# leaner-forever/SEGS-SLAM

Measured on AMD Instinct MI355X. Metric: mapper train-iters/sec (fwd+bwd raster), higher is better.
Workload: dtype f32; 1 GPU; 1080p_3m: 3000000 Gaussians, 1920x1080, 1 keyframe per GPU, fwd+bwd raster; P=3000000, P_visible=2096178, num_rendered=10472370, instances_binned=7913347, instances_live=6766534, width=1920, height=1080, parallelism=keyframe-dp1, forward=resident (no host sync), hipgraph=off

## Files before the change

### segs-slam_amd/csrc/binning.hip

```cpp
#include <hip/hip_runtime.h>
#include <cstdint>
#include "gs_layout.h"
#include "kernels.h"

namespace segs {

constexpr int PREFIX_ROWS = PREFIX_ROWS_PER_WG;

__global__ void __launch_bounds__(1024) scan_block_sums_kernel(uint32_t* __restrict__ block_sums, int nblocks,
                                                               const uint32_t* __restrict__ depth_range,
                                                               uint32_t* __restrict__ total) {
  __shared__ uint32_t w_sum[16], w_dmax[16], w_dnmin[16];
  const int tid = threadIdx.x, lane = tid & 63, wv = tid >> 6;
  uint32_t sum = 0, dmax = 0, dnmin = 0;
  for (int i = tid; i < nblocks; i += 1024) {
    sum += block_sums[i];
    dmax = max(dmax, depth_range[i]);
    dnmin = max(dnmin, depth_range[nblocks + i]);
  }
#pragma unroll
  for (int off = 32; off > 0; off >>= 1) {
    sum += __shfl_down(sum, off, 64);
    dmax = max(dmax, (uint32_t)__shfl_down((int)dmax, off, 64));
    dnmin = max(dnmin, (uint32_t)__shfl_down((int)dnmin, off, 64));
// ... 49 lines not shown
  __syncthreads();
  uint32_t carry = red[0] + red[1] + red[2] + red[3];
  uint32_t vals[PREFIX_ROWS];
#pragma unroll
  for (int r = 0; r < PREFIX_ROWS; r++) {
    const uint32_t slot = slot0 + (uint32_t)r * 256u + tid;
    vals[r] = slot < (uint32_t)P ? incl[slot] : 0u;
  }
#pragma unroll
  for (int r = 0; r < PREFIX_ROWS; r++) {
    const uint32_t slot = slot0 + (uint32_t)r * 256u + tid;
    uint32_t x = vals[r];
    const uint32_t t0 = x;
#pragma unroll
    for (int off = 1; off < 64; off <<= 1) {
      uint32_t y = __shfl_up(x, off, 64);
      if (lane >= off) x += y;
    }
    __syncthreads();
    if (lane == 63) wave_tot[wv] = x;
    __syncthreads();
    uint32_t base = carry;
    for (int w = 0; w < wv; w++) base += wave_tot[w];
    const uint32_t v = base + x;
    if (slot < (uint32_t)P) incl[slot] = v;
    if (slot < (uint32_t)P && first_owner && t0 != 0u) {
      const uint32_t excl = v - t0;
      for (uint32_t k = (excl + EMIT_SLOTS_PER_WG - 1) / EMIT_SLOTS_PER_WG; k * EMIT_SLOTS_PER_WG < v && k < owner_entries; k++)
        first_owner[k] = slot;
    }
    carry += wave_tot[0] + wave_tot[1] + wave_tot[2] + wave_tot[3];
  }
  if (total_out && blockIdx.x == gridDim.x - 1 && tid == 0) total_out[0] = carry;
}

constexpr int EMIT_SLOTS = EMIT_SLOTS_PER_WG;
static_assert(EMIT_SLOTS == 2 * 256, "two consecutive slots per thread");
struct EmitLds {
  uint32_t excl[EMIT_SLOTS + 2];
  uint32_t idx[EMIT_SLOTS + 1];
  uint2 bin[EMIT_SLOTS + 1];
  float4 geo0[EMIT_SLOTS + 1];
  float2 geo1[EMIT_SLOTS + 1];
  uint32_t mark[EMIT_SLOTS];
  uint32_t wave_max[4];
};
constexpr uint32_t EMIT_OWNER_MASK = 1023u;

__device__ __forceinline__ void emit_stage_owner(EmitLds& L, int k, uint32_t idx, const float4& e0, const float4& e1) {
  const uint32_t rmin = __float_as_uint(e1.z), rmax = __float_as_uint(e1.w);
  L.idx[k] = idx;
  L.bin[k] = make_uint2(rmin, (rmax & 0xFFFFu) - (rmin & 0xFFFFu));
  const float op = e1.y;
  L.geo0[k] = make_float4(e0.x, e0.y, -e0.z, -0.5f * e0.w);
  L.geo1[k] = make_float2(-e1.x, (op * 255.0f > 1.0f) ? __builtin_amdgcn_logf(255.0f * op) * 1.0001f + 1e-3f : -1.0f);
}
__device__ __forceinline__ void emit_mark_owner(uint32_t* mark, int k, uint32_t start, uint32_t s0, uint32_t tag) {
  const uint32_t pos = start > s0 ? start - s0 : 0u;
  if (pos < (uint32_t)EMIT_SLOTS) mark[pos] = (tag << 10) | (uint32_t)k;
}
__device__ __forceinline__ void emit_scan_begin(EmitLds& L, const uint32_t* mark, int tid, uint32_t& m0, uint32_t& incl) {
  const uint2 m = *reinterpret_cast<const uint2*>(mark + 2 * tid);
  m0 = m.x;
  uint32_t x = max(m.x, m.y);
#pragma unroll
  for (int off = 1; off < 64; off <<= 1) {
// ... 359 lines not shown
      if (AUX) aux_out[gp] = s_aux[lp];
      if constexpr (sizeof(K) == 4) {
        if (ranges_out != nullptr) {
          const K prev = lp > 0 ? s_keys[lp - 1] : ~k, next = lp + 1 < nout ? s_keys[lp + 1] : ~k;
          if (k != prev) atomicMin(&ranges_out[k].x, (uint32_t)gp);
          if (k != next) atomicMax(&ranges_out[k].y, (uint32_t)gp + 1u);
        }
      }
    }
  }
}

#define SEGS_INSTANTIATE_RADIX(K, BITS)                                                                                          \
  template __global__ void radix_count_kernel<K, BITS>(const K*, int, int, uint32_t, int, uint32_t*, uint32_t*, int, int,       \
                                                       const uint32_t*, int, int, int);                                                  \
  template __global__ void radix_scatter_kernel<K, BITS, false>(const K*, const uint32_t*, K*, uint32_t*, int, int, uint32_t, int, \
                                                                const uint32_t*, const uint32_t*, const uint32_t*, int, int,        \
                                                                const uint32_t*, int, uint32_t*, const uint32_t*, uint32_t*, int, int, int, \
                                                                uint2*, uint32_t*, uint32_t*, int);
SEGS_INSTANTIATE_RADIX(uint64_t, 8)
SEGS_INSTANTIATE_RADIX(uint32_t, 8)
SEGS_INSTANTIATE_RADIX(uint32_t, 9)
SEGS_INSTANTIATE_RADIX(uint32_t, 11)
#undef SEGS_INSTANTIATE_RADIX
#define SEGS_INSTANTIATE_AUX(BITS)                                                                                                     \
  template __global__ void radix_scatter_kernel<uint32_t, BITS, true>(const uint32_t*, const uint32_t*, uint32_t*, uint32_t*, int, int, \
                                                                      uint32_t, int, const uint32_t*, const uint32_t*, const uint32_t*, \
                                                                      int, int, const uint32_t*, int, uint32_t*, const uint32_t*, uint32_t*, int, int, int, \
                                                                      uint2*, uint32_t*, uint32_t*, int);
SEGS_INSTANTIATE_AUX(8)
SEGS_INSTANTIATE_AUX(9)
#undef SEGS_INSTANTIATE_AUX

__global__ void __launch_bounds__(256) identify_tile_ranges_kernel(int L, const uint32_t* __restrict__ keys,
                                                                   uint2* __restrict__ ranges, const uint32_t* __restrict__ n_dev,
                                                                   uint32_t* __restrict__ status, uint32_t* __restrict__ status_mirror,
                                                                   const uint32_t* __restrict__ n_live ) {
  static_assert(RANGE_KEYS_PER_THREAD == 4, "one uint4 per thread");
  const int idx = blockIdx.x * 256 + threadIdx.x;
  if (n_dev) {
    const uint32_t n = *n_dev;
    if (idx == 0 && status) {
      const uint32_t over = (n > (uint32_t)L || status[2] != 0u) ? 1u : 0u;
      status[2] = 0u;
      status[3] = over;
      const uint32_t live = n_live ? min(*n_live, min(n, (uint32_t)L)) : min(n, (uint32_t)L);
      status[1] = live;
      if (status_mirror) { status_mirror[0] = n; status_mirror[1] = live; status_mirror[3] = over; }
    }
    L = (int)min(n, (uint32_t)L);
  }
  if (n_live) L = (int)min(*n_live, (uint32_t)L);
  const int i0 = idx * RANGE_KEYS_PER_THREAD;
  if (i0 >= L) return;
  uint32_t k[RANGE_KEYS_PER_THREAD];
  if (i0 + RANGE_KEYS_PER_THREAD <= L) {
    const uint4 v = *reinterpret_cast<const uint4*>(keys + i0);
    k[0] = v.x; k[1] = v.y; k[2] = v.z; k[3] = v.w;
  } else {
#pragma unroll
    for (int q = 0; q < RANGE_KEYS_PER_THREAD; q++) k[q] = i0 + q < L ? keys[i0 + q] : 0u;
  }
  uint32_t prev = i0 > 0 ? keys[i0 - 1] : 0u;
#pragma unroll
  for (int q = 0; q < RANGE_KEYS_PER_THREAD; q++) {
    const int i = i0 + q;
// ... 120 lines not shown
```

### segs-slam_amd/csrc/capi.hip

```cpp
#include <hip/hip_runtime.h>
#include <cstdio>
#include <cstdlib>
#include <algorithm>
#include <cstring>
#include <string>
#include <vector>
#include "../../include/segs_raster.h"
#include "gs_layout.h"
#include "kernels.h"

using namespace segs;

namespace {
thread_local std::string g_err;
}
int segs::set_error(int code, const char* what) {
  g_err = what;
  return code;
}
int segs::set_hip_error(hipError_t e, const char* where) {
  g_err = std::string(where) + ": " + hipGetErrorString(e);
  return (int)e > 0 ? (int)e : 1;
}

namespace {

thread_local uint32_t g_flags = 0u;
thread_local uint32_t* g_status_mirror = nullptr;

int fail(int code, const char* what) { return segs::set_error(code, what); }
int hip_fail(hipError_t e, const char* where) { return segs::set_hip_error(e, where); }
#define HIP_TRY(expr)                                   \
  do {                                                  \
    hipError_t _e = (expr);                             \
    if (_e != hipSuccess) return hip_fail(_e, #expr);   \
  } while (0)
#define LAUNCH_TRY(name)                                \
  do {                                                  \
    hipError_t _e = hipGetLastError();                  \
    if (_e != hipSuccess) return hip_fail(_e, name);    \
  } while (0)

enum KernelId { K_PREPROCESS_FWD = 0, K_SCAN, K_DUPLICATE, K_RADIX_COUNT, K_RADIX_SCAN, K_RADIX_SCATTER, K_RANGES,
                K_RENDER_FWD, K_RENDER_BWD, K_PREPROCESS_BWD, K_MEMSET, K_COUNT };
const char* const kKernelNames[K_COUNT] = {"preprocess_fwd_kernel", "scan_block_sums_kernel", "duplicate_with_keys_kernel",
                                           "radix_count_kernel", "radix_scan_kernel", "radix_scatter_kernel",
                                           "identify_tile_ranges_kernel", "render_fwd_kernel", "render_bwd_kernel",
                                           "preprocess_bwd_kernel", "memset"};
struct Profiler {
  unsigned mask = 0;
  std::vector<hipEvent_t> pool;
  size_t used = 0;
  struct Span { int id; size_t e0, e1; };
  std::vector<Span> spans;
  double total_ms[K_COUNT] = {0};
  long count[K_COUNT] = {0};
  hipEvent_t get() {
    if (used == pool.size()) { hipEvent_t e; if (hipEventCreate(&e) != hipSuccess) return nullptr; pool.push_back(e); }
    return pool[used++];
  }
} g_prof;
struct ProfScope {
  int id; hipStream_t st; size_t e0 = 0; bool on;
  ProfScope(int id_, hipStream_t st_) : id(id_), st(st_), on((g_prof.mask >> id_) & 1u) {
    if (on) { e0 = g_prof.used; hipEvent_t e = g_prof.get(); if (e) (void)hipEventRecord(e, st); else on = false; }
  }
  ~ProfScope() {
    if (on) { size_t e1 = g_prof.used; hipEvent_t e = g_prof.get(); if (e) { (void)hipEventRecord(e, st); g_prof.spans.push_back({id, e0, e1}); } }
  }
};
#define PROF(id) ProfScope _prof_scope_##id(id, st)

uint32_t getHigherMsb(uint32_t n) {
  uint32_t msb = sizeof(n) * 4, step = msb;
  while (step > 1) {
    step /= 2;
    if (n >> msb) msb += step; else msb -= step;
  }
  if (n >> msb) msb++;
  return msb;
}
// ... 86 lines not shown
  float* gacc() const { return (float*)(base + L.gacc); }
  uint32_t* touched() const { return (uint32_t*)(base + L.touched); }
};
Geom geom_at(char* p, int P) { return Geom{geom_layout(P), align_ptr(p)}; }
Geom geom_at(char* p, int P, int rows) {
  Geom g{geom_layout(rows), align_ptr(p)};
  g.L.P = P;
  g.L.nblocks = (P + 255) / 256;
  return g;
}

int run_preprocess(const Geom& G, int P, int W, int H, const float* means3D, const float* colors, const float* opac,
                   const float* scales, float mod, const float* rots, const float* cov3D_precomp, const float* view,
                   const float* proj, float tan_fovx, float tan_fovy, int* radii, const float* shs, int D, int M,
                   const float* cam_pos, hipStream_t st, uint32_t* depth_keys = nullptr, uint32_t* depth_vals = nullptr,
                   uint2* ranges = nullptr, uint32_t extra_flags = 0u, uint32_t* depth_overflow = nullptr) {
  const float focal_y = H / (2.0f * tan_fovy);
  const float focal_x = W / (2.0f * tan_fovx);
  const uint32_t gx = (W + TILE_X - 1) / TILE_X, gy = (H + TILE_Y - 1) / TILE_Y;
  { PROF(K_PREPROCESS_FWD);
  preprocess_fwd_kernel<<<G.L.nblocks, 256, 0, st>>>(P, means3D, scales, mod, rots, opac, colors, cov3D_precomp, view,
                                                     proj, W, H, tan_fovx, tan_fovy, focal_x, focal_y, gx, gy, radii,
                                                     G.rec(), G.bin(), G.block_sums(), G.block_sums() + (G.L.nblocks + 1), shs, D, M, cam_pos,
                                                     G.clamped(), g_flags | extra_flags, depth_keys, depth_vals, ranges, (int)(gx * gy),
                                                     depth_overflow, G.touched());
  }
  LAUNCH_TRY("preprocess_fwd_kernel");
  return SEGS_OK;
}

int run_binning(const Geom& G, char* bin, const BinningLayout& BL, const GaussSortLayout& GS, uint2* ranges, int P, int n_cap,
                const uint32_t* n_dev, uint32_t dmin, int dbits, uint32_t dcull, uint32_t gx, uint32_t gy, uint32_t* total_out,
                hipStream_t st, bool depth_keys_ready = false, bool drop_dead = false, bool nine_bit_depth = false,
                const uint32_t* depth_keys_src = nullptr ) {
  const int bit = (int)getHigherMsb(gx * gy);
  char* gbin = bin + GS.base;
  const BinningLayout& GL = GS.inner;
  const int gside = (nine_bit_depth ? (dbits + 8) / 9 : (dbits + 7) / 8) & 1;
  if (!depth_keys_ready) { PROF(K_DUPLICATE);
  make_depth_keys_kernel<<<G.L.nblocks, 256, 0, st>>>(P, G.bin(), dcull, (uint32_t*)(gbin + GL.keys[gside]), (uint32_t*)(gbin + GL.vals[gside]),
                                                      ranges, (int)(gx * gy));
  }
  LAUNCH_TRY("make_depth_keys_kernel");
  const bool drop_culled = depth_keys_ready;
  int idx_bits = 1;
  while (idx_bits < 32 && ((uint64_t)1 << idx_bits) < (uint64_t)P) idx_bits++;
  int pack_shift = (32 - idx_bits >= 6 && !(g_flags & SEGS_RASTER_GATHER_TILES_TOUCHED)) ? idx_bits : 0;
  if (pack_shift && (g_flags & SEGS_RASTER_TEST_NARROW_PACK)) pack_shift = 30;
  uint32_t* aux_final = pack_shift ? nullptr : G.offsets();
  int rc = nine_bit_depth ? sort_pairs<uint32_t, 9>(gbin, GL, P, dbits, dmin, dbits, st, nullptr, drop_culled, true, G.touched(), aux_final, pack_shift, SortFusion(), depth_keys_src)
                          : sort_pairs<uint32_t>(gbin, GL, P, dbits, dmin, dbits, st, nullptr, drop_culled, true, G.touched(), aux_final, pack_shift, SortFusion(), depth_keys_src);
  if (rc) return rc;
  uint32_t* order = (uint32_t*)(gbin + GL.vals[0]);
  const uint32_t* ng_dev = drop_culled ? (const uint32_t*)(gbin + GL.n_live) : nullptr;
  uint32_t* sums2 = (uint32_t*)(bin + GS.block_sums);
  uint32_t* first_owner = (uint32_t*)(bin + GS.first_owner);
  const int prefix_wgs = (P + 256 * PREFIX_ROWS_PER_WG - 1) / (256 * PREFIX_ROWS_PER_WG);
  { PROF(K_SCAN);
  ordered_block_sums_kernel<<<prefix_wgs, 256, 0, st>>>(P, pack_shift ? G.touched() : G.offsets(), nullptr, sums2, G.offsets(), ng_dev, order, pack_shift);
  }
  LAUNCH_TRY("ordered_block_sums_kernel");
#ifdef SEGS_MEASURE
  static const bool no_wide = getenv("SEGS_NO_WIDE_DIGIT") != nullptr;
#else
  constexpr bool no_wide = false;
#endif
  const bool wide_digit = !no_wide && bit <= 11 && BL.nblocks <= SORT_WIDE_MAX_TILES;
  const int tpasses = wide_digit ? 1 : (bit + 7) / 8;
  const int side = tpasses & 1;
  { PROF(K_SCAN);
  ordered_offsets_kernel<<<prefix_wgs, 256, 0, st>>>(P, sums2, G.offsets(), total_out, ng_dev, first_owner,
                                                      (uint32_t)(n_cap / EMIT_SLOTS_PER_WG + 2));
  }
  LAUNCH_TRY("ordered_offsets_kernel");
  const bool unfused = (g_flags & SEGS_RASTER_UNFUSED_BINNING) != 0u;
  { PROF(K_DUPLICATE);
  duplicate_with_keys_kernel<<<(n_cap + EMIT_SLOTS_PER_WG - 1) / EMIT_SLOTS_PER_WG, 256, 0, st>>>(P, n_cap, G.rec(), order, G.offsets(),
                                                                    (uint32_t*)(bin + BL.keys[side]), (uint32_t*)(bin + BL.vals[side]), gx, n_dev,
                                                                    drop_dead ? 1 : 0, ng_dev, first_owner);
  }
  LAUNCH_TRY("duplicate_with_keys_kernel");
  SortFusion fuse;
  const bool fused_ranges = !unfused && tpasses >= 2;
  if (fused_ranges) {
    fuse.ranges = ranges;
    fuse.status = n_dev ? total_out : nullptr;
    fuse.status_mirror = n_dev ? g_status_mirror : nullptr;
    fuse.keep_sorted_keys = n_dev == nullptr;
  }
  rc = wide_digit ? sort_pairs<uint32_t, 11>(bin, BL, n_cap, bit, 0u, 0, st, n_dev, drop_dead, false, nullptr, nullptr, 0, fuse)
                  : sort_pairs<uint32_t>(bin, BL, n_cap, bit, 0u, 0, st, n_dev, drop_dead, false, nullptr, nullptr, 0, fuse);
  if (rc) return rc;
  if (!fused_ranges) { PROF(K_RANGES);
  identify_tile_ranges_kernel<<<(n_cap + 256 * RANGE_KEYS_PER_THREAD - 1) / (256 * RANGE_KEYS_PER_THREAD), 256, 0, st>>>(n_cap, (const uint32_t*)(bin + BL.keys[0]), ranges, n_dev,
                                                                   n_dev ? total_out : nullptr, n_dev ? g_status_mirror : nullptr,
                                                                   drop_dead ? (const uint32_t*)(bin + BL.n_live) : nullptr);
  }
  LAUNCH_TRY("identify_tile_ranges_kernel");
  return SEGS_OK;
}

int launch_render_fwd(uint32_t tiles, const uint2* ranges, const uint32_t* point_list, int width, int height, const float* rec,
                      const float* background, float* final_T, uint32_t* n_contrib, float* out_color, const segs_depth_outputs* dout,
                      hipStream_t st) {
  PROF(K_RENDER_FWD);
  if (dout && (dout->depth || dout->alpha))
    render_fwd_depth_kernel<<<tiles, 256, 0, st>>>(ranges, point_list, width, height, rec, background, final_T, n_contrib, out_color,
                                                   dout->depth, dout->alpha);
  else
    render_fwd_kernel<<<tiles, 256, 0, st>>>(ranges, point_list, width, height, rec, background, final_T, n_contrib, out_color);
  LAUNCH_TRY("render_fwd_kernel");
  return SEGS_OK;
}

}

extern "C" {

const char* segs_last_error(void) { return g_err.c_str(); }

uint32_t* segs_raster_set_status_mirror(uint32_t* host_mapped_status) {
  uint32_t* old = g_status_mirror;
  g_status_mirror = host_mapped_status;
  return old;
}

uint32_t segs_raster_set_flags(uint32_t flags) {
  const uint32_t old = g_flags;
  g_flags = flags;
  return old;
}
// ... 395 lines not shown
                                    const float* background, int width, int height, const float* means3D, const float* shs,
                                    const float* colors_precomp, const float* opacities, const float* scales, float scale_modifier,
                                    const float* rotations, const float* cov3D_precomp, const float* viewmatrix,
                                    const float* projmatrix, const float* cam_pos, float tan_fovx, float tan_fovy, float* out_color,
                                    int* radii, uint32_t* status, const segs_depth_outputs* dout, void* stream) {
  hipStream_t st = (hipStream_t)stream;
  if (P <= 0 || capacity <= 0 || width <= 0 || height <= 0) return fail(SEGS_ERR_INVALID_ARGUMENT, "bad sizes");
  if (geom_rows < P) return fail(SEGS_ERR_INVALID_ARGUMENT, "geom_rows (rows the geometry buffer was sized for) must be >= P");
  if (geom_rows > MAX_GAUSSIANS) return fail(SEGS_ERR_INVALID_ARGUMENT, "P exceeds 2^28 Gaussians");
  if (!geom_buffer || !binning_buffer || !image_buffer || !status || !background || !out_color || !viewmatrix || !projmatrix ||
      !means3D || !opacities)
    return fail(SEGS_ERR_INVALID_ARGUMENT, "null required pointer");
  if (!colors_precomp && (!shs || !cam_pos || M <= 0 || D < 0 || (D + 1) * (D + 1) > M || D > 3))
    return fail(SEGS_ERR_INVALID_ARGUMENT, "need colors_precomp, or shs + cam_pos with (D+1)^2 <= M, D <= 3");
  if (!cov3D_precomp && (!scales || !rotations)) return fail(SEGS_ERR_INVALID_ARGUMENT, "need scales+rotations or cov3D_precomp");
  const uint32_t gx = (width + TILE_X - 1) / TILE_X, gy = (height + TILE_Y - 1) / TILE_Y;
  if (gx > 0xFFFFu || gy > 0xFFFFu) return fail(SEGS_ERR_INVALID_ARGUMENT, "image too large for 16-bit tile coordinates");
  Geom G = geom_at(geom_buffer, P, geom_rows);
  char* img = align_ptr(image_buffer);
  char* bin = align_ptr(binning_buffer);
  const ImageLayout IL = image_layout(width, height);
  const BinningLayout BL = binning_layout(capacity);
  const GaussSortLayout GS = gauss_sort_layout(capacity, P);
  if (!radii) radii = G.radii_internal();
  uint2* ranges = (uint2*)(img + IL.ranges);
  char* gbin = bin + GS.base;
  const int gside = (3 & 1);
  int rc = run_preprocess(G, P, width, height, means3D, colors_precomp, opacities, cov3D_precomp ? nullptr : scales, scale_modifier,
                          rotations, cov3D_precomp, viewmatrix, projmatrix, tan_fovx, tan_fovy, radii, shs, D, M, cam_pos, st,
                          (uint32_t*)(gbin + GS.inner.keys[gside]), (uint32_t*)(gbin + GS.inner.vals[gside]), ranges,
                          (g_flags & SEGS_RASTER_KEEP_DEAD_INSTANCES) ? 0u : PREPROCESS_TIGHT_RECT, status + 2);
  if (rc) return rc;
  rc = run_binning(G, bin, BL, GS, ranges, P, capacity, status, DEPTH_KEY_MIN, DEPTH_KEY_BITS, 0xFFFFFFFFu, gx, gy, status, st, true,
                   (g_flags & SEGS_RASTER_KEEP_DEAD_INSTANCES) == 0u, true);
  if (rc) return rc;
  return launch_render_fwd(gx * gy, ranges, (const uint32_t*)(bin + BL.vals[0]), width, height, G.rec(), background,
                           (float*)(img + IL.final_T), (uint32_t*)(img + IL.n_contrib), out_color, dout, st);
}

int segs_rasterize_forward_resident(char* geom_buffer, char* binning_buffer, char* image_buffer, int capacity, int geom_rows, int P, int D, int M,
                                    const float* background, int width, int height, const float* means3D, const float* shs,
                                    const float* colors_precomp, const float* opacities, const float* scales, float scale_modifier,
                                    const float* rotations, const float* cov3D_precomp, const float* viewmatrix,
                                    const float* projmatrix, const float* cam_pos, float tan_fovx, float tan_fovy, float* out_color,
                                    int* radii, uint32_t* status, void* stream) {
  return rasterize_forward_resident_impl(geom_buffer, binning_buffer, image_buffer, capacity, geom_rows, P, D, M, background, width, height,
                                         means3D, shs, colors_precomp, opacities, scales, scale_modifier, rotations, cov3D_precomp,
                                         viewmatrix, projmatrix, cam_pos, tan_fovx, tan_fovy, out_color, radii, status, nullptr, stream);
}

int segs_rasterize_forward_resident_depth(char* geom_buffer, char* binning_buffer, char* image_buffer, int capacity, int geom_rows, int P,
                                          int D, int M, const float* background, int width, int height, const float* means3D,
                                          const float* shs, const float* colors_precomp, const float* opacities, const float* scales,
                                          float scale_modifier, const float* rotations, const float* cov3D_precomp,
                                          const float* viewmatrix, const float* projmatrix, const float* cam_pos, float tan_fovx,
                                          float tan_fovy, float* out_color, int* radii, uint32_t* status,
                                          const segs_depth_outputs* depth_out, void* stream) {
  return rasterize_forward_resident_impl(geom_buffer, binning_buffer, image_buffer, capacity, geom_rows, P, D, M, background, width, height,
                                         means3D, shs, colors_precomp, opacities, scales, scale_modifier, rotations, cov3D_precomp,
                                         viewmatrix, projmatrix, cam_pos, tan_fovx, tan_fovy, out_color, radii, status, depth_out, stream);
}

int segs_resident_projection_targets(char* geom_buffer, char* binning_buffer, char* image_buffer, int capacity, int geom_rows, int P,
                                     int width, int height, int* radii, uint32_t* status, segs_projection_targets* out) {
  if (P <= 0 || capacity <= 0 || width <= 0 || height <= 0 || !out) return fail(SEGS_ERR_INVALID_ARGUMENT, "bad sizes");
  if (geom_rows < P) return fail(SEGS_ERR_INVALID_ARGUMENT, "geom_rows (rows the geometry buffer was sized for) must be >= P");
  if (geom_rows > MAX_GAUSSIANS) return fail(SEGS_ERR_INVALID_ARGUMENT, "P exceeds 2^28 Gaussians");
// ... 4 lines not shown
  const ImageLayout IL = image_layout(width, height);
  const GaussSortLayout GS = gauss_sort_layout(capacity, P);
  const int gside = (3 & 1);
  out->records = G.rec();
  out->radii = radii ? radii : G.radii_internal();
  out->tiles_touched = G.touched();
  out->depth_keys = (uint32_t*)(align_ptr(binning_buffer) + GS.base + GS.inner.keys[gside]);
  out->tile_ranges = (uint32_t*)(align_ptr(image_buffer) + IL.ranges);
  out->depth_overflow = status + 2;
  out->num_tiles = (int)(gx * gy);
  out->flags = (g_flags & SEGS_RASTER_KEEP_DEAD_INSTANCES) ? 0u : PREPROCESS_TIGHT_RECT;
  return SEGS_OK;
}

static int rasterize_forward_resident_projected_impl(char* geom_buffer, char* binning_buffer, char* image_buffer, int capacity,
                                                    int geom_rows, int P, const float* background, int width, int height, float* out_color,
                                                    uint32_t* status, const segs_depth_outputs* dout, void* stream) {
  hipStream_t st = (hipStream_t)stream;
  if (P <= 0 || capacity <= 0 || width <= 0 || height <= 0) return fail(SEGS_ERR_INVALID_ARGUMENT, "bad sizes");
  if (geom_rows < P) return fail(SEGS_ERR_INVALID_ARGUMENT, "geom_rows (rows the geometry buffer was sized for) must be >= P");
  if (geom_rows > MAX_GAUSSIANS) return fail(SEGS_ERR_INVALID_ARGUMENT, "P exceeds 2^28 Gaussians");
  if (!geom_buffer || !binning_buffer || !image_buffer || !status || !background || !out_color)
    return fail(SEGS_ERR_INVALID_ARGUMENT, "null required pointer");
  const uint32_t gx = (width + TILE_X - 1) / TILE_X, gy = (height + TILE_Y - 1) / TILE_Y;
  if (gx > 0xFFFFu || gy > 0xFFFFu) return fail(SEGS_ERR_INVALID_ARGUMENT, "image too large for 16-bit tile coordinates");
  Geom G = geom_at(geom_buffer, P, geom_rows);
  char* img = align_ptr(image_buffer);
  char* bin = align_ptr(binning_buffer);
  const ImageLayout IL = image_layout(width, height);
  const BinningLayout BL = binning_layout(capacity);
  const GaussSortLayout GS = gauss_sort_layout(capacity, P);
  uint2* ranges = (uint2*)(img + IL.ranges);
  int rc = run_binning(G, bin, BL, GS, ranges, P, capacity, status, DEPTH_KEY_MIN, DEPTH_KEY_BITS, 0xFFFFFFFFu, gx, gy, status, st, true,
                       (g_flags & SEGS_RASTER_KEEP_DEAD_INSTANCES) == 0u, true);
  if (rc) return rc;
  return launch_render_fwd(gx * gy, ranges, (const uint32_t*)(bin + BL.vals[0]), width, height, G.rec(), background,
                           (float*)(img + IL.final_T), (uint32_t*)(img + IL.n_contrib), out_color, dout, st);
}

int segs_rasterize_forward_resident_projected(char* geom_buffer, char* binning_buffer, char* image_buffer, int capacity, int geom_rows, int P,
                                              const float* background, int width, int height, float* out_color, uint32_t* status,
                                              void* stream) {
  return rasterize_forward_resident_projected_impl(geom_buffer, binning_buffer, image_buffer, capacity, geom_rows, P, background, width,
                                                   height, out_color, status, nullptr, stream);
}

int segs_rasterize_forward_resident_projected_depth(char* geom_buffer, char* binning_buffer, char* image_buffer, int capacity,
                                                    int geom_rows, int P, const float* background, int width, int height,
                                                    float* out_color, uint32_t* status, const segs_depth_outputs* depth_out,
                                                    void* stream) {
  return rasterize_forward_resident_projected_impl(geom_buffer, binning_buffer, image_buffer, capacity, geom_rows, P, background, width,
                                                   height, out_color, status, depth_out, stream);
}

int segs_rasterize_backward_resident(char* geom_buffer, char* binning_buffer, char* image_buffer, int capacity, int geom_rows, int P, int D, int M,
                                     const float* background, int width, int height, const float* means3D, const float* shs,
                                     const float* scales, float scale_modifier, const float* rotations, const float* cov3D_precomp,
                                     const float* viewmatrix, const float* projmatrix, const float* campos, float tan_fovx,
                                     float tan_fovy, const int* radii, const float* dL_dpix, float* dL_dmean2D, float* dL_dconic,
                                     float* dL_dopacity, float* dL_dcolor, float* dL_dmean3D, float* dL_dcov3D, float* dL_dsh,
                                     float* dL_dscale, float* dL_drot, void* stream) {
  return rasterize_backward_impl(P, D, M, capacity, background, width, height, means3D, shs, scales, scale_modifier, rotations,
                                 cov3D_precomp, viewmatrix, projmatrix, campos, tan_fovx, tan_fovy, radii, geom_buffer, binning_buffer,
                                 image_buffer, dL_dpix, dL_dmean2D, dL_dconic, dL_dopacity, dL_dcolor, dL_dmean3D, dL_dcov3D, dL_dsh,
                                 dL_dscale, dL_drot, stream, true, geom_rows, nullptr);
}

// ... 40 lines not shown
```

### segs-slam_amd/csrc/kernels.h

```cpp
#pragma once
#include <hip/hip_runtime.h>
#include <cstdint>
#include "gs_layout.h"

namespace segs {

int set_error(int code, const char* what);
int set_hip_error(hipError_t e, const char* where);


__global__ void preprocess_fwd_kernel(
    int P, const float* __restrict__ means3D, const float* __restrict__ scales, float mod,
    const float* __restrict__ rotations, const float* __restrict__ opacities, const float* __restrict__ colors,
    const float* __restrict__ cov3D_precomp, const float* __restrict__ viewmatrix, const float* __restrict__ projmatrix,
    int W, int H, float tan_fovx, float tan_fovy, float focal_x, float focal_y, uint32_t gx, uint32_t gy,
    int* __restrict__ radii, float* __restrict__ rec, BinInfo* __restrict__ bin, uint32_t* __restrict__ block_sums,
    uint32_t* __restrict__ depth_range, const float* __restrict__ shs, int D, int M, const float* __restrict__ cam_pos,
    uint32_t* __restrict__ clamped, uint32_t flags, uint32_t* __restrict__ depth_keys, uint32_t* __restrict__ depth_vals,
    uint2* __restrict__ ranges, int num_tiles, uint32_t* __restrict__ depth_overflow, uint32_t* __restrict__ touched_dense);
constexpr uint32_t DEPTH_KEY_MIN = 0x3E4CCCCDu;
constexpr int DEPTH_KEY_BITS = 27;

__global__ void visible_filter_kernel(
    int P, const float* __restrict__ means3D, const float* __restrict__ scales, float mod,
    const float* __restrict__ rotations, const float* __restrict__ cov3D_precomp,
    const float* __restrict__ viewmatrix, const float* __restrict__ projmatrix, int W, int H,
    float tan_fovx, float tan_fovy, float focal_x, float focal_y, uint32_t gx, uint32_t gy, int* __restrict__ radii,
    int log_scale_stride);

__global__ void mark_visible_kernel(int P, const float* __restrict__ means3D, const float* __restrict__ viewmatrix,
                                    uint8_t* __restrict__ present);

template <bool DEPTH>
__global__ void preprocess_bwd_kernel(
    int P, const float* __restrict__ means3D, const int* __restrict__ radii, const float* __restrict__ scales,
    const float* __restrict__ rotations, float mod, const float* __restrict__ cov3D_precomp,
    const float* __restrict__ view, const float* __restrict__ proj, float h_x, float h_y, float tan_fovx, float tan_fovy,
    float* __restrict__ gacc, float img_w, float img_h,
    float* __restrict__ dL_dmean2D, float* __restrict__ dL_dconic,
    float* __restrict__ dL_dopacity, float* __restrict__ dL_dcolor, float* __restrict__ dL_dmean3D,
    float* __restrict__ dL_dcov3D, float* __restrict__ dL_dscale, float* __restrict__ dL_drot, int clean_gacc);
__global__ void sh_backward_kernel(int P, const float* __restrict__ means3D, const int* __restrict__ radii,
                                   const float* __restrict__ shs, int D, int M, const float* __restrict__ cam_pos,
                                   const uint32_t* __restrict__ clamped, const float* __restrict__ dL_dcolor,
                                   float* __restrict__ dL_dmean3D, float* __restrict__ dL_dsh);

__global__ void scan_block_sums_kernel(uint32_t* __restrict__ block_sums, int nblocks, const uint32_t* __restrict__ depth_range,
                                       uint32_t* __restrict__ total);
__global__ void ordered_offsets_kernel(int P, const uint32_t* __restrict__ block_sums, uint32_t* __restrict__ incl,
                                       uint32_t* __restrict__ total_out, const uint32_t* __restrict__ ng_dev,
                                       uint32_t* __restrict__ first_owner, uint32_t owner_entries);
__global__ void duplicate_with_keys_kernel(int P, int R, const float* __restrict__ rec,
                                           const uint32_t* __restrict__ order, const uint32_t* __restrict__ incl,
                                           uint32_t* __restrict__ keys, uint32_t* __restrict__ vals, uint32_t gx,
                                           const uint32_t* __restrict__ n_dev, int mark_dead, const uint32_t* __restrict__ ng_dev,
                                           const uint32_t* __restrict__ first_owner);
constexpr uint32_t RANGE_EMPTY_START = 0xFFFFFFFFu;
__global__ void normalize_ranges_kernel(int num_tiles, uint2* __restrict__ ranges);
constexpr uint32_t PREPROCESS_TIGHT_RECT = 0x80000000u;
constexpr uint32_t DEAD_KEY = 0xFFFFFFFFu;
template <typename K, int BITS>
__global__ void radix_count_kernel(const K* __restrict__ keys, int n, int shift, uint32_t dmin, int dbits,
                                   uint32_t* __restrict__ tile_prefix, uint32_t* __restrict__ chunk_hist, int nblocks, int nchunks,
                                   const uint32_t* __restrict__ n_dev, int drop_dead, int chunk_tiles, int nbits);
__global__ void radix_scan_kernel(uint32_t* __restrict__ block_hist, int nblocks, uint32_t* __restrict__ digit_totals);
template <typename K, int BITS, bool AUX>
__global__ void radix_scatter_kernel(const K* __restrict__ keys_in, const uint32_t* __restrict__ vals_in,
                                     K* __restrict__ keys_out, uint32_t* __restrict__ vals_out, int n, int shift,
                                     uint32_t dmin, int dbits, const uint32_t* __restrict__ tile_prefix, const uint32_t* __restrict__ chunk_prefix,
                                     const uint32_t* __restrict__ digit_totals, int nblocks, int nchunks,
                                     const uint32_t* __restrict__ n_dev, int drop_dead, uint32_t* __restrict__ n_live_out,
                                     const uint32_t* __restrict__ aux_in, uint32_t* __restrict__ aux_out, int nbits, int chunk_tiles, int pack_shift,
                                     uint2* __restrict__ ranges_out, uint32_t* __restrict__ status, uint32_t* __restrict__ status_mirror,
                                     int write_keys);
__global__ void identify_tile_ranges_kernel(int L, const uint32_t* __restrict__ keys, uint2* __restrict__ ranges,
                                            const uint32_t* __restrict__ n_dev, uint32_t* __restrict__ status,
                                            uint32_t* __restrict__ status_mirror, const uint32_t* __restrict__ n_live);

__global__ void render_fwd_kernel(const uint2* __restrict__ ranges, const uint32_t* __restrict__ point_list, int W, int H,
                                  const float* __restrict__ rec, const float* __restrict__ bg,
                                  float* __restrict__ final_T, uint32_t* __restrict__ n_contrib, float* __restrict__ out_color);
__global__ void render_bwd_kernel(const uint2* __restrict__ ranges, const uint32_t* __restrict__ point_list, int W, int H,
                                  const float* __restrict__ rec, const float* __restrict__ bg,
                                  const float* __restrict__ final_T, const uint32_t* __restrict__ n_contrib,
// ... 32 lines not shown
```

Measured before the change: 1002 iters/s.

## Replace global depth sort with index-order binning plus per-tile depth sort

Instead of radix-sorting all visible Gaussians by depth before duplication, Gaussians are compacted in index order with a fused count/offset scan. After tile binning, a new kernel sorts each tile's instance list by depth in LDS, using a chunked merge-rank path for large tiles. This removes the global depth sort passes in exchange for per-tile sorting work and extra key gathers, which may be imbalanced on heavy tiles.

New measurement: 1016 iters/s, median of 6. +1.3%, better.

```diff
diff --git a/segs-slam_amd/csrc/binning.hip b/segs-slam_amd/csrc/binning.hip
--- a/segs-slam_amd/csrc/binning.hip
+++ b/segs-slam_amd/csrc/binning.hip
@@ -105,6 +105,75 @@
     carry += wave_tot[0] + wave_tot[1] + wave_tot[2] + wave_tot[3];
   }
   if (total_out && blockIdx.x == gridDim.x - 1 && tid == 0) total_out[0] = carry;
+}
+
+__global__ void __launch_bounds__(256) index_block_sums_kernel(int P, const uint32_t* __restrict__ touched,
+                                                               uint32_t* __restrict__ block_sums, uint32_t* __restrict__ block_owners) {
+  __shared__ uint32_t wave_sums[4], wave_owners[4];
+  uint32_t s = 0, c = 0;
+#pragma unroll
+  for (int r = 0; r < PREFIX_ROWS; r++) {
+    const int g = (blockIdx.x * PREFIX_ROWS + r) * 256 + threadIdx.x;
+    const uint32_t v = g < P ? touched[g] : 0u;
+    s += v;
+    c += v != 0u ? 1u : 0u;
+  }
+#pragma unroll
+  for (int off = 32; off > 0; off >>= 1) { s += __shfl_down(s, off, 64); c += __shfl_down(c, off, 64); }
+  if ((threadIdx.x & 63) == 0) { wave_sums[threadIdx.x >> 6] = s; wave_owners[threadIdx.x >> 6] = c; }
+  __syncthreads();
+  if (threadIdx.x == 0) {
+    block_sums[blockIdx.x] = wave_sums[0] + wave_sums[1] + wave_sums[2] + wave_sums[3];
+    block_owners[blockIdx.x] = wave_owners[0] + wave_owners[1] + wave_owners[2] + wave_owners[3];
+  }
+}
+__global__ void __launch_bounds__(256) index_offsets_kernel(int P, const uint32_t* __restrict__ touched, const uint32_t* __restrict__ block_sums,
+                                                            const uint32_t* __restrict__ block_owners, uint32_t* __restrict__ order,
+                                                            uint32_t* __restrict__ incl, uint32_t* __restrict__ total_out, uint32_t* __restrict__ ng_out,
+                                                            uint32_t* __restrict__ first_owner, uint32_t owner_entries) {
+  __shared__ uint32_t wave_tot[4], wave_cnt[4], red[4], red_c[4];
+  const int tid = threadIdx.x, lane = tid & 63, wv = tid >> 6;
+  uint32_t before = 0, before_c = 0;
+  for (int b = tid; b < (int)blockIdx.x; b += 256) { before += block_sums[b]; before_c += block_owners[b]; }
+#pragma unroll
+  for (int off = 32; off > 0; off >>= 1) { before += __shfl_down(before, off, 64); before_c += __shfl_down(before_c, off, 64); }
+  if (lane == 0) { red[wv] = before; red_c[wv] = before_c; }
+  __syncthreads();
+  uint32_t carry = red[0] + red[1] + red[2] + red[3], carry_c = red_c[0] + red_c[1] + red_c[2] + red_c[3];
+  const int g0 = blockIdx.x * 256 * PREFIX_ROWS;
+  uint32_t vals[PREFIX_ROWS];
+#pragma unroll
+  for (int r = 0; r < PREFIX_ROWS; r++) {
+    const int g = g0 + r * 256 + tid;
+    vals[r] = g < P ? touched[g] : 0u;
+  }
+#pragma unroll
+  for (int r = 0; r < PREFIX_ROWS; r++) {
+    const int g = g0 + r * 256 + tid;
+    const uint32_t t0 = vals[r];
+    uint32_t x = t0, c = t0 != 0u ? 1u : 0u;
+#pragma unroll
+    for (int off = 1; off < 64; off <<= 1) {
+      const uint32_t y = __shfl_up(x, off, 64), yc = __shfl_up(c, off, 64);
+      if (lane >= off) { x += y; c += yc; }
+    }
+    __syncthreads();
+    if (lane == 63) { wave_tot[wv] = x; wave_cnt[wv] = c; }
+    __syncthreads();
+    uint32_t base = carry, base_c = carry_c;
+    for (int w = 0; w < wv; w++) { base += wave_tot[w]; base_c += wave_cnt[w]; }
+    if (t0 != 0u) {
+      const uint32_t v = base + x, slot = base_c + c - 1u;
+      order[slot] = (uint32_t)g;
+      incl[slot] = v;
+      const uint32_t excl = v - t0;
+      for (uint32_t k = (excl + EMIT_SLOTS_PER_WG - 1) / EMIT_SLOTS_PER_WG; k * EMIT_SLOTS_PER_WG < v && k < owner_entries; k++)
+        first_owner[k] = slot;
+    }
+    carry += wave_tot[0] + wave_tot[1] + wave_tot[2] + wave_tot[3];
+    carry_c += wave_cnt[0] + wave_cnt[1] + wave_cnt[2] + wave_cnt[3];
+  }
+  if (blockIdx.x == gridDim.x - 1 && tid == 0) { total_out[0] = carry; ng_out[0] = carry_c; }
 }
 
 constexpr int EMIT_SLOTS = EMIT_SLOTS_PER_WG;
@@ -530,6 +599,188 @@
 SEGS_INSTANTIATE_AUX(9)
 #undef SEGS_INSTANTIATE_AUX
 
+constexpr int TILE_ORDER_CAP = SORT_TILE;
+constexpr int TILE_ORDER_ITEMS = SORT_ITEMS_PER_THREAD;
+constexpr int TO_BITS = 9, TO_DIGITS = 1 << TO_BITS;
+struct TileOrderLds {
+  uint32_t key[TILE_ORDER_CAP];
+  uint32_t val[TILE_ORDER_CAP];
+  uint32_t cnt[4][TO_DIGITS];
+  uint32_t start[TO_DIGITS];
+  uint32_t red[8];
+};
+__device__ __forceinline__ int tile_order_block(int n) { return ((n + 255) >> 8) * 64; }
+
+__device__ void tile_order_sort(TileOrderLds& L, uint32_t (&key)[TILE_ORDER_ITEMS], uint32_t (&val)[TILE_ORDER_ITEMS], int n) {
+  const int tid = threadIdx.x, lane = tid & 63, wv = tid >> 6;
+  const int blk = tile_order_block(n), wave_base = wv * blk;
+  uint32_t kmin = 0xFFFFFFFFu, kmax = 0u;
+#pragma unroll
+  for (int r = 0; r < TILE_ORDER_ITEMS; r++)
+    if (r * 64 < blk && wave_base + r * 64 + lane < n) { kmin = min(kmin, key[r]); kmax = max(kmax, key[r]); }
+#pragma unroll
+  for (int off = 32; off > 0; off >>= 1) {
+    kmin = min(kmin, (uint32_t)__shfl_xor((int)kmin, off, 64));
+    kmax = max(kmax, (uint32_t)__shfl_xor((int)kmax, off, 64));
+  }
+  if (lane == 0) { L.red[wv] = kmin; L.red[4 + wv] = kmax; }
+  __syncthreads();
+  kmin = min(min(L.red[0], L.red[1]), min(L.red[2], L.red[3]));
+  kmax = max(max(L.red[4], L.red[5]), max(L.red[6], L.red[7]));
+  const uint32_t span = kmax - kmin;
+  const int bits = span ? 32 - __clz((int)span) : 0;
+  const int passes = (bits + TO_BITS - 1) / TO_BITS;
+  if (passes == 0) {
+#pragma unroll
+    for (int r = 0; r < TILE_ORDER_ITEMS; r++) {
+      const int i = wave_base + r * 64 + lane;
+      if (r * 64 < blk && i < n) { L.key[i] = key[r]; L.val[i] = val[r]; }
+    }
+    __syncthreads();
+    return;
+  }
+  volatile uint32_t* my = L.cnt[wv];
+  for (int p = 0; p < passes; p++) {
+    const int shift = TO_BITS * p, nbits = min(TO_BITS, bits - shift);
+#pragma unroll
+    for (int w = 0; w < 4; w++) { L.cnt[w][tid] = 0u; L.cnt[w][tid + 256] = 0u; }
+    __syncthreads();
+    uint32_t drank[TILE_ORDER_ITEMS];
+#pragma unroll
+    for (int r = 0; r < TILE_ORDER_ITEMS; r++) {
+      drank[r] = 0xFFFFFFFFu;
+      if (r * 64 >= blk || wave_base + r * 64 >= n) continue;
+      const bool valid = wave_base + r * 64 + lane < n;
+      const uint32_t d = valid ? ((key[r] - kmin) >> shift) & (TO_DIGITS - 1u) : 0u;
+      const uint64_t peers = match_digit<TO_BITS>(d, __ballot(valid), nbits);
+      const uint32_t below = mbcnt(peers);
+      uint32_t old = 0;
+      if (valid) old = my[d];
+      __builtin_amdgcn_wave_barrier();
+      if (valid && below == 0) my[d] = old + (uint32_t)__popcll(peers);
+      __builtin_amdgcn_wave_barrier();
+      if (valid) drank[r] = d | ((old + below) << TO_BITS);
+    }
+    __syncthreads();
+    uint32_t run0 = 0, run1 = 0;
+#pragma unroll
+    for (int w = 0; w < 4; w++) {
+      const uint2 c = *reinterpret_cast<const uint2*>(&L.cnt[w][2 * tid]);
+      *reinterpret_cast<uint2*>(&L.cnt[w][2 * tid]) = make_uint2(run0, run1);
+      run0 += c.x; run1 += c.y;
+    }
+    const uint32_t run = run0 + run1;
+    uint32_t x = run;
+#pragma unroll
+    for (int off = 1; off < 64; off <<= 1) {
+      const uint32_t y = __shfl_up(x, off, 64);
+      if (lane >= off) x += y;
+    }
+    if (lane == 63) L.red[wv] = x;
+    __syncthreads();
+    uint32_t base = 0;
+    for (int w = 0; w < wv; w++) base += L.red[w];
+    *reinterpret_cast<uint2*>(&L.start[2 * tid]) = make_uint2(base + x - run, base + x - run1);
+    __syncthreads();
+#pragma unroll
+    for (int r = 0; r < TILE_ORDER_ITEMS; r++) {
+      if (drank[r] != 0xFFFFFFFFu) {
+        const uint32_t d = drank[r] & (TO_DIGITS - 1u);
+        const uint32_t pos = L.start[d] + L.cnt[wv][d] + (drank[r] >> TO_BITS);
+        L.key[pos] = key[r];
+        L.val[pos] = val[r];
+      }
+    }
+    __syncthreads();
+    if (p + 1 < passes) {
+#pragma unroll
+      for (int r = 0; r < TILE_ORDER_ITEMS; r++) {
+        const int i = wave_base + r * 64 + lane;
+        if (r * 64 < blk && i < n) { key[r] = L.key[i]; val[r] = L.val[i]; }
+      }
+    }
+  }
+}
+
+__device__ __forceinline__ void tile_order_load(uint32_t (&key)[TILE_ORDER_ITEMS], uint32_t (&val)[TILE_ORDER_ITEMS],
+                                                const uint32_t* __restrict__ vals, const uint32_t* __restrict__ depth_keys, int n) {
+  const int blk = tile_order_block(n), wave_base = (threadIdx.x >> 6) * blk, lane = threadIdx.x & 63;
+#pragma unroll
+  for (int r = 0; r < TILE_ORDER_ITEMS; r++) {
+    const int i = wave_base + r * 64 + lane;
+    val[r] = (r * 64 < blk && i < n) ? vals[i] : 0u;
+  }
+#pragma unroll
+  for (int r = 0; r < TILE_ORDER_ITEMS; r++) {
+    const int i = wave_base + r * 64 + lane;
+    key[r] = (r * 64 < blk && i < n) ? depth_keys[val[r] & ID_MASK] : 0u;
+  }
+}
+
+__global__ void __launch_bounds__(256) tile_depth_order_kernel(const uint2* __restrict__ ranges, int num_tiles, uint32_t* __restrict__ vals,
+                                                               const uint32_t* __restrict__ depth_keys, uint32_t* __restrict__ park_keys,
+                                                               uint32_t* __restrict__ park_vals, uint32_t capacity) {
+  __shared__ TileOrderLds L;
+  const int tiles_per_xcd = (num_tiles + 7) >> 3;
+  const int tile = (int)(blockIdx.x & 7u) * tiles_per_xcd + (int)(blockIdx.x >> 3);
+  if ((int)(blockIdx.x >> 3) >= tiles_per_xcd || tile >= num_tiles) return;
+  const uint2 rg = ranges[tile];
+  if (rg.x >= rg.y || rg.y > capacity) return;
+  const int n = (int)(rg.y - rg.x);
+  if (n <= 1) return;
+  uint32_t* tv = vals + rg.x;
+  uint32_t key[TILE_ORDER_ITEMS], val[TILE_ORDER_ITEMS];
+  const int tid = threadIdx.x;
+  if (n <= TILE_ORDER_CAP) {
+    tile_order_load(key, val, tv, depth_keys, n);
+    tile_order_sort(L, key, val, n);
+    for (int i = tid; i < n; i += 256) tv[i] = L.val[i];
+    return;
+  }
+  uint32_t* pk = park_keys + rg.x;
+  uint32_t* pv = park_vals + rg.x;
+  const int nchunks = (n + TILE_ORDER_CAP - 1) / TILE_ORDER_CAP;
+  for (int c = 0; c < nchunks; c++) {
+    const int c0 = c * TILE_ORDER_CAP, cn = min(TILE_ORDER_CAP, n - c0);
+    tile_order_load(key, val, tv + c0, depth_keys, cn);
+    tile_order_sort(L, key, val, cn);
+    for (int i = tid; i < cn; i += 256) { pk[c0 + i] = L.key[i]; pv[c0 + i] = L.val[i]; }
+    __syncthreads();
+  }
+  const int wave_base = (tid >> 6) * (TILE_ORDER_CAP / 4), lane = tid & 63;
+  for (int a = 0; a < nchunks; a++) {
+    const int a0 = a * TILE_ORDER_CAP, an = min(TILE_ORDER_CAP, n - a0);
+    uint32_t rank[TILE_ORDER_ITEMS];
+#pragma unroll
+    for (int r = 0; r < TILE_ORDER_ITEMS; r++) {
+      const int i = wave_base + r * 64 + lane;
+      key[r] = i < an ? pk[a0 + i] : 0u;
+      val[r] = i < an ? pv[a0 + i] : 0u;
+      rank[r] = (uint32_t)i;
+    }
+    for (int b = 0; b < nchunks; b++) {
+      if (b == a) continue;
+      const int b0 = b * TILE_ORDER_CAP, bn = min(TILE_ORDER_CAP, n - b0);
+      __syncthreads();
+      for (int i = tid; i < bn; i += 256) L.key[i] = pk[b0 + i];
+      __syncthreads();
+#pragma unroll
+      for (int r = 0; r < TILE_ORDER_ITEMS; r++) {
+        const uint64_t k = (uint64_t)key[r] + (b < a ? 1u : 0u);
+        int lo = 0, hi = bn;
+        while (lo < hi) {
+          const int mid = (lo + hi) >> 1;
+          if ((uint64_t)L.key[mid] < k) lo = mid + 1; else hi = mid;
+        }
+        rank[r] += (uint32_t)lo;
+      }
+    }
+#pragma unroll
+    for (int r = 0; r < TILE_ORDER_ITEMS; r++)
+      if (wave_base + r * 64 + lane < an) tv[rank[r]] = val[r];
+  }
+}
+
 __global__ void __launch_bounds__(256) identify_tile_ranges_kernel(int L, const uint32_t* __restrict__ keys,
                                                                    uint2* __restrict__ ranges, const uint32_t* __restrict__ n_dev,
                                                                    uint32_t* __restrict__ status, uint32_t* __restrict__ status_mirror,
diff --git a/segs-slam_amd/csrc/capi.hip b/segs-slam_amd/csrc/capi.hip
--- a/segs-slam_amd/csrc/capi.hip
+++ b/segs-slam_amd/csrc/capi.hip
@@ -42,11 +42,11 @@
   } while (0)
 
 enum KernelId { K_PREPROCESS_FWD = 0, K_SCAN, K_DUPLICATE, K_RADIX_COUNT, K_RADIX_SCAN, K_RADIX_SCATTER, K_RANGES,
-                K_RENDER_FWD, K_RENDER_BWD, K_PREPROCESS_BWD, K_MEMSET, K_COUNT };
+                K_RENDER_FWD, K_RENDER_BWD, K_PREPROCESS_BWD, K_MEMSET, K_TILE_ORDER, K_COUNT };
 const char* const kKernelNames[K_COUNT] = {"preprocess_fwd_kernel", "scan_block_sums_kernel", "duplicate_with_keys_kernel",
                                            "radix_count_kernel", "radix_scan_kernel", "radix_scatter_kernel",
                                            "identify_tile_ranges_kernel", "render_fwd_kernel", "render_bwd_kernel",
-                                           "preprocess_bwd_kernel", "memset"};
+                                           "preprocess_bwd_kernel", "memset", "tile_depth_order_kernel"};
 struct Profiler {
   unsigned mask = 0;
   std::vector<hipEvent_t> pool;
@@ -199,34 +199,52 @@
 int run_binning(const Geom& G, char* bin, const BinningLayout& BL, const GaussSortLayout& GS, uint2* ranges, int P, int n_cap,
                 const uint32_t* n_dev, uint32_t dmin, int dbits, uint32_t dcull, uint32_t gx, uint32_t gy, uint32_t* total_out,
                 hipStream_t st, bool depth_keys_ready = false, bool drop_dead = false, bool nine_bit_depth = false,
-                const uint32_t* depth_keys_src = nullptr ) {
+                const uint32_t* depth_keys_src = nullptr ,
+                bool tile_order = false ) {
   const int bit = (int)getHigherMsb(gx * gy);
   char* gbin = bin + GS.base;
   const BinningLayout& GL = GS.inner;
   const int gside = (nine_bit_depth ? (dbits + 8) / 9 : (dbits + 7) / 8) & 1;
-  if (!depth_keys_ready) { PROF(K_DUPLICATE);
-  make_depth_keys_kernel<<<G.L.nblocks, 256, 0, st>>>(P, G.bin(), dcull, (uint32_t*)(gbin + GL.keys[gside]), (uint32_t*)(gbin + GL.vals[gside]),
-                                                      ranges, (int)(gx * gy));
-  }
-  LAUNCH_TRY("make_depth_keys_kernel");
-  const bool drop_culled = depth_keys_ready;
-  int idx_bits = 1;
-  while (idx_bits < 32 && ((uint64_t)1 << idx_bits) < (uint64_t)P) idx_bits++;
-  int pack_shift = (32 - idx_bits >= 6 && !(g_flags & SEGS_RASTER_GATHER_TILES_TOUCHED)) ? idx_bits : 0;
-  if (pack_shift && (g_flags & SEGS_RASTER_TEST_NARROW_PACK)) pack_shift = 30;
-  uint32_t* aux_final = pack_shift ? nullptr : G.offsets();
-  int rc = nine_bit_depth ? sort_pairs<uint32_t, 9>(gbin, GL, P, dbits, dmin, dbits, st, nullptr, drop_culled, true, G.touched(), aux_final, pack_shift, SortFusion(), depth_keys_src)
-                          : sort_pairs<uint32_t>(gbin, GL, P, dbits, dmin, dbits, st, nullptr, drop_culled, true, G.touched(), aux_final, pack_shift, SortFusion(), depth_keys_src);
-  if (rc) return rc;
-  uint32_t* order = (uint32_t*)(gbin + GL.vals[0]);
-  const uint32_t* ng_dev = drop_culled ? (const uint32_t*)(gbin + GL.n_live) : nullptr;
+  const int prefix_wgs = (P + 256 * PREFIX_ROWS_PER_WG - 1) / (256 * PREFIX_ROWS_PER_WG);
   uint32_t* sums2 = (uint32_t*)(bin + GS.block_sums);
   uint32_t* first_owner = (uint32_t*)(bin + GS.first_owner);
-  const int prefix_wgs = (P + 256 * PREFIX_ROWS_PER_WG - 1) / (256 * PREFIX_ROWS_PER_WG);
-  { PROF(K_SCAN);
-  ordered_block_sums_kernel<<<prefix_wgs, 256, 0, st>>>(P, pack_shift ? G.touched() : G.offsets(), nullptr, sums2, G.offsets(), ng_dev, order, pack_shift);
-  }
-  LAUNCH_TRY("ordered_block_sums_kernel");
+  uint32_t* order = (uint32_t*)(gbin + GL.vals[0]);
+  const uint32_t* ng_dev = nullptr;
+  int rc = SEGS_OK;
+  if (tile_order) {
+    uint32_t* owners = sums2 + prefix_wgs;
+    uint32_t* ng = (uint32_t*)(gbin + GL.n_live);
+    { PROF(K_SCAN);
+    index_block_sums_kernel<<<prefix_wgs, 256, 0, st>>>(P, G.touched(), sums2, owners);
+    }
+    LAUNCH_TRY("index_block_sums_kernel");
+    { PROF(K_SCAN);
+    index_offsets_kernel<<<prefix_wgs, 256, 0, st>>>(P, G.touched(), sums2, owners, order, G.offsets(), total_out, ng, first_owner,
+                                                     (uint32_t)(n_cap / EMIT_SLOTS_PER_WG + 2));
+    }
+    LAUNCH_TRY("index_offsets_kernel");
+    ng_dev = ng;
+  } else {
+    if (!depth_keys_ready) { PROF(K_DUPLICATE);
+    make_depth_keys_kernel<<<G.L.nblocks, 256, 0, st>>>(P, G.bin(), dcull, (uint32_t*)(gbin + GL.keys[gside]), (uint32_t*)(gbin + GL.vals[gside]),
+                                                        ranges, (int)(gx * gy));
+    }
+    LAUNCH_TRY("make_depth_keys_kernel");
+    const bool drop_culled = depth_keys_ready;
+    int idx_bits = 1;
+    while (idx_bits < 32 && ((uint64_t)1 << idx_bits) < (uint64_t)P) idx_bits++;
+    int pack_shift = (32 - idx_bits >= 6 && !(g_flags & SEGS_RASTER_GATHER_TILES_TOUCHED)) ? idx_bits : 0;
+    if (pack_shift && (g_flags & SEGS_RASTER_TEST_NARROW_PACK)) pack_shift = 30;
+    uint32_t* aux_final = pack_shift ? nullptr : G.offsets();
+    rc = nine_bit_depth ? sort_pairs<uint32_t, 9>(gbin, GL, P, dbits, dmin, dbits, st, nullptr, drop_culled, true, G.touched(), aux_final, pack_shift, SortFusion(), depth_keys_src)
+                          : sort_pairs<uint32_t>(gbin, GL, P, dbits, dmin, dbits, st, nullptr, drop_culled, true, G.touched(), aux_final, pack_shift, SortFusion(), depth_keys_src);
+    if (rc) return rc;
+    ng_dev = drop_culled ? (const uint32_t*)(gbin + GL.n_live) : nullptr;
+    { PROF(K_SCAN);
+    ordered_block_sums_kernel<<<prefix_wgs, 256, 0, st>>>(P, pack_shift ? G.touched() : G.offsets(), nullptr, sums2, G.offsets(), ng_dev, order, pack_shift);
+    }
+    LAUNCH_TRY("ordered_block_sums_kernel");
+  }
 #ifdef SEGS_MEASURE
   static const bool no_wide = getenv("SEGS_NO_WIDE_DIGIT") != nullptr;
 #else
@@ -235,11 +253,13 @@
   const bool wide_digit = !no_wide && bit <= 11 && BL.nblocks <= SORT_WIDE_MAX_TILES;
   const int tpasses = wide_digit ? 1 : (bit + 7) / 8;
   const int side = tpasses & 1;
-  { PROF(K_SCAN);
-  ordered_offsets_kernel<<<prefix_wgs, 256, 0, st>>>(P, sums2, G.offsets(), total_out, ng_dev, first_owner,
-                                                      (uint32_t)(n_cap / EMIT_SLOTS_PER_WG + 2));
-  }
-  LAUNCH_TRY("ordered_offsets_kernel");
+  if (!tile_order) {
+    { PROF(K_SCAN);
+    ordered_offsets_kernel<<<prefix_wgs, 256, 0, st>>>(P, sums2, G.offsets(), total_out, ng_dev, first_owner,
+                                                        (uint32_t)(n_cap / EMIT_SLOTS_PER_WG + 2));
+    }
+    LAUNCH_TRY("ordered_offsets_kernel");
+  }
   const bool unfused = (g_flags & SEGS_RASTER_UNFUSED_BINNING) != 0u;
   { PROF(K_DUPLICATE);
   duplicate_with_keys_kernel<<<(n_cap + EMIT_SLOTS_PER_WG - 1) / EMIT_SLOTS_PER_WG, 256, 0, st>>>(P, n_cap, G.rec(), order, G.offsets(),
@@ -264,6 +284,15 @@
                                                                    drop_dead ? (const uint32_t*)(bin + BL.n_live) : nullptr);
   }
   LAUNCH_TRY("identify_tile_ranges_kernel");
+  if (tile_order) {
+    const int tiles = (int)(gx * gy);
+    { PROF(K_TILE_ORDER);
+    tile_depth_order_kernel<<<(tiles + 7) / 8 * 8, 256, 0, st>>>(ranges, tiles, (uint32_t*)(bin + BL.vals[0]),
+                                                                 (const uint32_t*)(gbin + GL.keys[gside]), (uint32_t*)(bin + BL.keys[1]),
+                                                                 (uint32_t*)(bin + BL.vals[1]), (uint32_t)n_cap);
+    }
+    LAUNCH_TRY("tile_depth_order_kernel");
+  }
   return SEGS_OK;
 }
 
@@ -725,7 +754,7 @@
                           (g_flags & SEGS_RASTER_KEEP_DEAD_INSTANCES) ? 0u : PREPROCESS_TIGHT_RECT, status + 2);
   if (rc) return rc;
   rc = run_binning(G, bin, BL, GS, ranges, P, capacity, status, DEPTH_KEY_MIN, DEPTH_KEY_BITS, 0xFFFFFFFFu, gx, gy, status, st, true,
-                   (g_flags & SEGS_RASTER_KEEP_DEAD_INSTANCES) == 0u, true);
+                   (g_flags & SEGS_RASTER_KEEP_DEAD_INSTANCES) == 0u, true, nullptr, true);
   if (rc) return rc;
   return launch_render_fwd(gx * gy, ranges, (const uint32_t*)(bin + BL.vals[0]), width, height, G.rec(), background,
                            (float*)(img + IL.final_T), (uint32_t*)(img + IL.n_contrib), out_color, dout, st);
@@ -796,7 +825,7 @@
   const GaussSortLayout GS = gauss_sort_layout(capacity, P);
   uint2* ranges = (uint2*)(img + IL.ranges);
   int rc = run_binning(G, bin, BL, GS, ranges, P, capacity, status, DEPTH_KEY_MIN, DEPTH_KEY_BITS, 0xFFFFFFFFu, gx, gy, status, st, true,
-                       (g_flags & SEGS_RASTER_KEEP_DEAD_INSTANCES) == 0u, true);
+                       (g_flags & SEGS_RASTER_KEEP_DEAD_INSTANCES) == 0u, true, nullptr, true);
   if (rc) return rc;
   return launch_render_fwd(gx * gy, ranges, (const uint32_t*)(bin + BL.vals[0]), width, height, G.rec(), background,
                            (float*)(img + IL.final_T), (uint32_t*)(img + IL.n_contrib), out_color, dout, st);
diff --git a/segs-slam_amd/csrc/kernels.h b/segs-slam_amd/csrc/kernels.h
--- a/segs-slam_amd/csrc/kernels.h
+++ b/segs-slam_amd/csrc/kernels.h
@@ -50,6 +50,15 @@
 __global__ void ordered_offsets_kernel(int P, const uint32_t* __restrict__ block_sums, uint32_t* __restrict__ incl,
                                        uint32_t* __restrict__ total_out, const uint32_t* __restrict__ ng_dev,
                                        uint32_t* __restrict__ first_owner, uint32_t owner_entries);
+__global__ void index_block_sums_kernel(int P, const uint32_t* __restrict__ touched, uint32_t* __restrict__ block_sums,
+                                        uint32_t* __restrict__ block_owners);
+__global__ void index_offsets_kernel(int P, const uint32_t* __restrict__ touched, const uint32_t* __restrict__ block_sums,
+                                     const uint32_t* __restrict__ block_owners, uint32_t* __restrict__ order, uint32_t* __restrict__ incl,
+                                     uint32_t* __restrict__ total_out, uint32_t* __restrict__ ng_out, uint32_t* __restrict__ first_owner,
+                                     uint32_t owner_entries);
+__global__ void tile_depth_order_kernel(const uint2* __restrict__ ranges, int num_tiles, uint32_t* __restrict__ vals,
+                                        const uint32_t* __restrict__ depth_keys, uint32_t* __restrict__ park_keys,
+                                        uint32_t* __restrict__ park_vals, uint32_t capacity);
 __global__ void duplicate_with_keys_kernel(int P, int R, const float* __restrict__ rec,
                                            const uint32_t* __restrict__ order, const uint32_t* __restrict__ incl,
                                            uint32_t* __restrict__ keys, uint32_t* __restrict__ vals, uint32_t gx,
```
